# NorESMhub/BLOM

Measured on AMD Instinct MI355X. Metric: simulated-days/sec, higher is better.
Workload: dtype f64; 1 GPU; channel 208x512x53 as 1 tile(s) of 208x512x53 along i, 1 tile per GPU, isopyc_bulkml/remap/geopotential/uc/enscon, ntr=3 (TKE, length-scale slot, ideal age: the reference default build), baclin=900s batrop=18s lstep=50; config 2's step (phy/mod_blom_step.F90:96-253: init_fluxes, tmsmt1, cmnfld2, difest_isobml [the whole routine: diffusivities estimated every step (NorESM defaults incl. rhsctp; the; physics=full, forcing=default, spinup_steps=0

## Files before the change

### blom_amd/csrc/blomgpu_internal.h

```cpp
#pragma once
#include <hip/hip_runtime.h>
#include <cstdint>
#include <string>
#include <unordered_map>
#include <vector>
#include "exp_libm.h"

#define NBDY 4

#ifdef BLOM_HOSTEMU
#define WAIT_VMCNT0() ((void)0)
#else
#define WAIT_VMCNT0() asm volatile("s_waitcnt vmcnt(0)" ::: "memory")
#endif

#define BLOM_REAL_FIELDS(X)                                                              \
                                                                          \
  X(u, 2 * K) X(v, 2 * K) X(dp, 2 * K) X(dpu, 2 * K) X(dpv, 2 * K) X(temp, 2 * K)        \
  X(saln, 2 * K) X(sigma, 2 * K) X(uflx, 2 * K) X(vflx, 2 * K) X(utflx, 2 * K)           \
  X(vtflx, 2 * K) X(usflx, 2 * K) X(vsflx, 2 * K)                                        \
  X(p, K + 1) X(pu, K + 1) X(pv, K + 1) X(phi, K + 1) X(cau, K) X(cav, K)                \
  X(ubflxs, 3) X(vbflxs, 3) X(ub, 2) X(vb, 2) X(pb, 2) X(pbu, 2) X(pbv, 2)               \
  X(ubflxs_p, 2) X(vbflxs_p, 2) X(pb_p, 1) X(pbu_p, 1) X(pbv_p, 1) X(ubcors_p, 1)        \
  X(vbcors_p, 1) X(sealv, 1)                                                             \
// ... 220 lines not shown
  bool ale_density_pc_upper = false, ale_density_pc_lower = false;
  int ale_regrid_method = 2, ale_k_range_plevel = 1;
  double ale_regrid_nudge_ts = 86400., ale_stab_fac_limit = .75, ale_dpvar_fac = .75, ale_smooth_diff_max = 50000.;
  int ale_dktzu = 4, ale_dktzl = 2;
  double ale_dpmin_interior = .1 * 9806.;
  int ndiff_rec_per_face = 0;
  int ndiff_surface_align = 1;
  double rm0 = 1.2, rm5 = 0., niwgf = 0., niwbf = .35, niwlf = .5;
  std::string mlrttp = "constant";
  double trxday = 0., srxday = 0., trxdpt = 1., srxdpt = 1., trxlim = 1.5, srxlim = .5, sref = 34.65, area = 0., xmi = 0.;
  int lmi[5] = {11, 12, 1, 2, 3};
  bool aptflx = false, apsflx = false, ditflx = false, disflx = false, srxbal = false;
  int ntda = 0;
  double swamxd = 200., brine_mlbase_frac = 0.;
  int mlrmth = 1;
  double eddtra_ce = .06, tau_mlr = 86400., tau_growing_hbl = 300., tau_decaying_hbl = 86400., tau_growing_hml = 3600.,
         tau_decaying_hml = 259200., lfmin = 5.e3, mlbl_max_ratio = 3., eddtra_cl = .25, mstar = .5, nstar = .066, wpup_min = 1.e-3;
  double egc = 0., eggam = 200., eglsmn = 4000., egmndf = 0., egmxdf = 1500., egidfq = 1., rhiscf = 0., ri0 = 1.2, tkepf = 0.;
  double bdml_logc = 0.;
  int eddf2d = 0, edsprs = 1, edanis = 0, redi3d = 0, rhsctp = 0, edfsmo = 0;
  int edritp_opt = 2, edwmth_opt = 1;
  bool smtfrc = false, use_stream_relaxation = false;
  int nstep_in_cpl = 1, l1ci = 1, l2ci = 1, nstep_in_day = 1, nday_of_year = 1;
  int cesm_single_sums = 0;
  bool full_physics = false;
  int difest_live = 0;
  int live_slopes = 0;
  int cmnfld1 = 0;
  int eddtra_frozen = 0;
  int check_period = 8;
  bool timing = false;
  int use_graph = 0;
  int overlap = 1;
  int phys_dag = 7;
  int mom_early_at = 0;
  int lean_fluxes = 1;
  int tmsmt_fold = 1;
  int tmsmt_ahead = 1;
  int remap_fold = 0;
  int remap_nfirst = 4;
  int halo_overlap = 1;
  int barotp_fused = 1;
  int barotp_tile = 0;
  int barotp_persist = 1;
  int barotp_block = 1;
  int barotp_overlap = 0;
  int barotp_rimbuf = 1;
  int barotp_arctic_persist = 1;
  int barotp_arctic_fused = 1;
  int arctic_strips = 0;
  int pgf_uv_pair = 0;
  int pgf_uv_ring = 7;
  int pgf_reuse = 0;
  int pgf_copy_fused = 1;
  int scan_reassoc = 0;
  int mom_aw_split = 0;
  int mom_force_aw = 0;
  int momtum_order = 0;
  int momtum_lds_pad = 0;
  int momtum_bs = 0;
  int momtum_chunks_a = 0, momtum_chunks_b = 0;
  int convec_nsingle = 2;
  int cmn_nslope_nb = 4;
  int diapfl_du = 8;
  int diffus_shfl = 0;
  int kprof_sel = 1;

// ... 220 lines not shown
```

### blom_amd/csrc/stage_cmnfld.hip

```cpp
#include "blomgpu_internal.h"
#include "eos.h"

#define GRAV 9.806
#define RHO0 1.e3
#define EPSILP 1.e-12
#define ONEM 9806.
#define ONEMM 9.806
#define SLS0 (10. * ONEM)
#define SLSMFQ 2.
#define SLSELS 2.
#define BFSQMN 1.e-7

enum { CM_DELP, CM_BFSQ, CM_SLS2, CM_GAM_ALE, CM_GAM = 9, CM_NSLOT };

#define COLUMN_IJ(V)                                                     \
  const int t_ = blockIdx.x * blockDim.x + threadIdx.x;                  \
  if (t_ >= (V).nplane) return;                                          \
  const int i = t_ % (V).ni - (NBDY - 1), j = t_ / (V).ni - (NBDY - 1);  \
  const size_t c = t_

__global__ __launch_bounds__(64) void k_cmn_bfsqf(const DevView *__restrict__ Vp, int n, int nn) {
  const DevView &V = *Vp;
  COLUMN_IJ(V);
  if (j < -1 || j > V.jj + 2 || i < -1 || i > V.ii + 2 || !V.m[I_ip][c]) return;
// ... 118 lines not shown
  L(bfsqf, kk + 1) = f_kk;
#undef L
}

__global__ __launch_bounds__(64) void k_cmn_phi(const DevView *__restrict__ Vp, int nn) {
  const DevView &V = *Vp;
  COLUMN_IJ(V);
  if (j < -1 || j > V.jj + 2 || i < -1 || i > V.ii + 2 || !V.m[I_ip][c]) return;
  const size_t np = V.nplane;
  const int kk = V.kk;
  gcd_t p = V.f[F_p] + c, temp = V.f[F_temp] + c + (size_t)nn * np, saln = V.f[F_saln] + c + (size_t)nn * np;
  gcd_t dp = V.f[F_dp] + c + (size_t)nn * np;
  gd_t phi = V.f[F_phi] + c;
  double ph = phi[(size_t)kk * np], plo = p[(size_t)kk * np];
  for (int k0 = kk - 1; k0 >= 0; k0 -= COLUMN_U) {
    double a[COLUMN_U], b[COLUMN_U], d[COLUMN_U], e[COLUMN_U];
#pragma unroll
    for (int u = 0; u < COLUMN_U; u++) {
      const size_t o = (size_t)(k0 - u >= 0 ? k0 - u : 0) * np;
      a[u] = p[o]; b[u] = dp[o]; d[u] = temp[o]; e[u] = saln[o];
    }
#pragma unroll
    for (int u = 0; u < COLUMN_U; u++) {
      const int k = k0 - u;
      if (k >= 0) {
        if (!(b[u] < EPSILP)) ph = ph - eos::p_alpha(plo, a[u], d[u], e[u]);
        phi[(size_t)k * np] = ph;
        plo = a[u];
      }
    }
  }
}

template <int NB>
__global__ __launch_bounds__(64) void k_cmn_nslope(const DevView *__restrict__ Vp, int n, int nn) {
  const DevView &V = *Vp;
  COLUMN_IJ(V);
  const bool isv = blockIdx.y == 1;
  if (isv ? (j < 0 || j > V.jj + 2 || i < -1 || i > V.ii + 2 || !V.m[I_iv][c])
          : (j < -1 || j > V.jj + 2 || i < 0 || i > V.ii + 2 || !V.m[I_iu][c])) return;
  const size_t np = V.nplane, a_ = isv ? c - V.ni : c - 1, b_ = c;
  const int kk = V.kk;
  gcd_t p = V.f[F_p], phi = V.f[F_phi], bf = V.f[F_bfsqf];
  gcd_t temp = V.f[F_temp] + (size_t)nn * np, saln = V.f[F_saln] + (size_t)nn * np, dp = V.f[F_dp] + (size_t)nn * np;
  gd_t nslp = (isv ? V.f[F_nslpy] : V.f[F_nslpx]) + c, nnslp = (isv ? V.f[F_nnslpy] : V.f[F_nnslpx]) + c;
  const double sci = (isv ? V.f[F_scvyi] : V.f[F_scuxi])[c];
#define A(f, x, k) (f)[(x) + (size_t)((k)-1) * np]
#define O(f, k) (f)[(size_t)((k)-1) * np]
  for (int k = 1; k <= kk; k++) { O(nslp, k) = 0.; O(nnslp, k) = 0.; }
  const int kfa = V.m[I_kfpla][a_ + (size_t)(n - 1) * np], kfb = V.m[I_kfpla][b_ + (size_t)(n - 1) * np];
  if (!(kfa <= kk || kfb <= kk)) return;
  int kmax = 1;
  for (int k0 = 3; k0 <= kk; k0 += COLUMN_U) {
    double da[COLUMN_U], db[COLUMN_U];
#pragma unroll
    for (int u = 0; u < COLUMN_U; u++) { const int kq = k0 + u <= kk ? k0 + u : kk; da[u] = A(dp, a_, kq); db[u] = A(dp, b_, kq); }
#pragma unroll
    for (int u = 0; u < COLUMN_U; u++)
      if (k0 + u <= kk && (da[u] > EPSILP || db[u] > EPSILP)) kmax = k0 + u;
  }
  const int kintr = kfa > kfb ? kfa : kfb;
  int knnsl = 2;
  const double phba = A(phi, a_, kk + 1), phbb = A(phi, b_, kk + 1);
  {
    const double pm = .5 * (A(p, a_, 3) + A(p, b_, 3));
    const double rx = eos::rho(pm, A(temp, b_, 2), A(saln, b_, 2)) - eos::rho(pm, A(temp, a_, 2), A(saln, a_, 2));
// ... 12 lines not shown
#pragma unroll
      for (int u = 0; u < NB; u++) {
        const int kq = k0 + u <= kmax ? k0 + u : kmax;
        pa[u] = A(p, a_, kq); pb[u] = A(p, b_, kq);
        tb[u] = A(temp, b_, kq); sb[u] = A(saln, b_, kq); ta[u] = A(temp, a_, kq); sa[u] = A(saln, a_, kq);
        fb[u] = A(phi, b_, kq); fa[u] = A(phi, a_, kq); ba[u] = A(bf, a_, kq); bb[u] = A(bf, b_, kq);
      }
#pragma unroll
      for (int u = 0; u < NB; u++) {
        const int k = k0 + u;
        if (k > kmax) break;
        const double pm = .5 * (pa[u] + pb[u]);
        const double rx = .5 * (eos::rho(pm, tbm, sbm) - eos::rho(pm, tam, sam) + eos::rho(pm, tb[u], sb[u]) - eos::rho(pm, ta[u], sa[u]));
        const double px = fb[u] - fa[u];
        const double bm = .5 * (ba[u] + bb[u]);
        const double s = (GRAV * rx / (RHO0 * bm) + px / GRAV) * sci;
        O(nslp, k) = s;
        if (fb[u] > phba && fa[u] > phbb) { O(nnslp, k) = sqrt(bm) * s; knnsl = k; }
        tbm = tb[u]; sbm = sb[u]; tam = ta[u]; sam = sa[u];
      }
    }
  }
  {
    const double last = O(nnslp, knnsl);
    for (int k = knnsl + 1; k <= kmax; k++) O(nnslp, k) = last;
  }
  if (kintr < kmax) {
    const double s = O(nslp, kintr + 1), ns = O(nnslp, kintr + 1);
    for (int k = 4; k <= kintr; k++) { O(nslp, k) = s; O(nnslp, k) = ns; }
  } else {
    const double s = O(nslp, 3), ns = O(nnslp, 3);
    for (int k = 4; k <= kmax; k++) { O(nslp, k) = s; O(nnslp, k) = ns; }
  }
#undef A
#undef O
}

__global__ __launch_bounds__(64) void k_cmn_z(const DevView *__restrict__ Vp, int mm) {
  const DevView &V = *Vp;
  COLUMN_IJ(V);
  if (j < 1 || j > V.jj || i < 1 || i > V.ii || !V.m[I_ip][c]) return;
  const size_t np = V.nplane;
  const int kk = V.kk;
  gcd_t p = V.f[F_p] + c, temp = V.f[F_temp] + c + (size_t)mm * np, saln = V.f[F_saln] + c + (size_t)mm * np;
  gcd_t dp = V.f[F_dp] + c + (size_t)mm * np;
  gd_t z = V.f[F_z] + c, dz = V.f[F_dz] + c;
  double zlo = -V.f[F_phi][c + (size_t)kk * np] / GRAV, plo = p[(size_t)kk * np];
  z[(size_t)kk * np] = zlo;
  for (int k0 = kk - 1; k0 >= 0; k0 -= COLUMN_U) {
    double a[COLUMN_U], b[COLUMN_U], d[COLUMN_U], e[COLUMN_U];
#pragma unroll
    for (int u = 0; u < COLUMN_U; u++) {
      const size_t o = (size_t)(k0 - u >= 0 ? k0 - u : 0) * np;
      a[u] = p[o]; b[u] = dp[o]; d[u] = temp[o]; e[u] = saln[o];
    }
#pragma unroll
    for (int u = 0; u < COLUMN_U; u++) {
      const int k = k0 - u;
      if (k < 0) break;
      const double zk = b[u] < EPSILP ? zlo : zlo + eos::p_alpha(plo, a[u], d[u], e[u]) / GRAV;
      z[(size_t)k * np] = zk;
      dz[(size_t)k * np] = zlo - zk;
      zlo = zk; plo = a[u];
    }
  }
}
// ... 307 lines not shown
    if (int rc = st_xctilr_multi(c, 2, ptrs, nl, 3, 3, it)) return rc;
  }
  const dim3 g1 = plane_grid(h, 1, 64), g2 = plane_grid(h, 2, 64);
  if (h.P.vcoord_tag != 1) {
    if (h.P.ltedtp_opt == 2 && h.P.eitmth == 2) {
      if (int rc = st_xctilr(c, h.f[F_nslpx], 1, h.kk, 2, 2, 13)) return rc;
      if (int rc = st_xctilr(c, h.f[F_nslpy], 1, h.kk, 2, 2, 14)) return rc;
    }
    TimeScope ts(c, "cmnfld");
    HIPCHK(c, hipMemsetAsync(h.f[F_bfsqi], 0, sizeof(double) * (size_t)(h.kk + 1) * h.nplane, c->stream));
    HIPCHK(c, hipMemsetAsync(h.f[F_bfsql], 0, sizeof(double) * (size_t)h.kk * h.nplane, c->stream));
    hipLaunchKernelGGL(k_cmn_bfsqf_ale, g1, dim3(64), 0, c->stream, c->d, nn);
    if (h.P.eitmth == 2) {
      if (h.P.ltedtp_opt == 2) hipLaunchKernelGGL(k_cmn_nnslope_ale, g2, dim3(64), 0, c->stream, c->d);
      else {
        hipLaunchKernelGGL(k_cmn_phi, g1, dim3(64), 0, c->stream, c->d, nn);
        hipLaunchKernelGGL(k_cmn_nslope_ale, g2, dim3(64), 0, c->stream, c->d, nn);
      }
    }
    HIPCHK(c, hipGetLastError());
    return 0;
  }
  if (int rc = st_kfpla_halo(c, n)) return rc;
  if (h.P.eitmth != 2) return 0;
  const bool aside = ctx_overlap_on(c) && (c->phys_dag & 1) && !c->tiling.multi();
  hipStream_t s = c->stream;
  if (aside) {
    if (int rc = launch_pscan(c, nn, -2, 3)) return rc;
    c->seq.pscan_done_ahead = true;
    if (int rc = ctx_side_fork(c, 4)) return rc;
    s = c->side;
  }
  TimeScope ts(c, "cmnfld");
  hipLaunchKernelGGL(k_cmn_bfsqf, g1, dim3(64), 0, s, c->d, n, nn);
  hipLaunchKernelGGL(k_cmn_phi, g1, dim3(64), 0, s, c->d, nn);
  switch (c->cmn_nslope_nb) {
    case 4: hipLaunchKernelGGL(k_cmn_nslope<4>, g2, dim3(64), 0, s, c->d, n, nn); break;
    case 3: hipLaunchKernelGGL(k_cmn_nslope<3>, g2, dim3(64), 0, s, c->d, n, nn); break;
    default: hipLaunchKernelGGL(k_cmn_nslope<2>, g2, dim3(64), 0, s, c->d, n, nn); break;
  }
  HIPCHK(c, hipGetLastError());
  c->seq.cmn_on_side = aside;
  return 0;
}
```

### blom_amd/csrc/stage_difest_iso.hip

```cpp
#include "blomgpu_internal.h"
#include "../../include/blomgpu.h"
#include "eos.h"
#include "pow_libm.h"
#include "sin_libm.h"
#include "atan2_libm.h"
#include <cmath>

#define PLANE_IJ(V)                                                        \
  unsigned bx_, by_;                                                       \
  xcd_block(bx_, by_);                                                     \
  const int t_ = bx_ * blockDim.x + threadIdx.x;                           \
  (void)by_;                                                               \
  if (t_ >= (V).nplane) return;                                            \
  const int i = t_ % (V).ni - (NBDY - 1), j = t_ / (V).ni - (NBDY - 1);    \
  const size_t c = t_;                                                     \
  (void)i; (void)j; (void)c

#define GRAV 9.806
#define ALPHA0 1.e-3
#define PI_BLOM 3.1415926536
#define BU 8
#define EPSILP 1.e-12
#define ONEM 9806.
#define DPBMIN 98.06
// ... 13 lines not shown
#define DPGRAV (100. * ONEM)
#define DPDIAV (100. * ONEM)
#define DPDDAV (10. * ONEM)
#define DPNBAV (250. * ONEM)
#define USTMIN .001
#define KAPPA .4
#define BFEPS 1.e-16
#define SLEPS .1
#define ZETAS (-1.)
#define CPSEMIN (-0.2)
#define URMSEMIN 0.05
#define AS_ (-28.86)
#define CS_ 98.96
#define GLS_CMU0 .527
#define PR_T 1.
#define GLS_C1 1.44
#define GLS_C2 1.92
#define GLS_C3PLUS 1.
#define GLS_C3MINUS (-.63)
#define GLS_GH0 .0329
#define GLS_GHMIN (-.28)
#define GLS_GHCRI .03
#define LS_UNLMT_MIN 1.e-8

enum { W_DU2 = 0, W_DV2, W_BVFSQ, W_BVF, W_EGR, W_ANISOK, W_SM1, W_SM2, W_NUB, W_NSLOT };

struct TkeC {
  double sqrt2, cmu_fac1, cmu_fac2, cmu_fac3, tke_exp1, gls_exp1, gls_fac6, s0, s1, s2, s4, s5, s6, b0, b1, b2, b3, b4, b5, cmu0p3;
  double gls_qfac, gls_bbc, gls_cmu0p;
};
struct DfePar {
  double egc, eggam, eglsmn, egmndf, egmxdf, egidfq, rhiscf, ri0, tkepf, niwgf, niwbf, niwlf, bdml_logc;
  int eddf2d, edsprs, edanis, redi3d, edritp, edwmth, use_tke, use_gls, itke, igls, rhsctp;
  TkeC T;
};

static TkeC tke_consts() {
  const double L1 = .107, L2 = .0032, L3 = .0864, L4 = .12, L5 = 11.9, L6 = .4, L7 = .0, L8 = .48;
  const double gls_p = 3., gls_m = 1.5, gls_n = -1.;
  TkeC t;
  t.sqrt2 = std::sqrt(2.);
  t.cmu_fac1 = std::pow(GLS_CMU0, -gls_p / gls_n);
  t.cmu_fac2 = std::pow(GLS_CMU0, 3. + gls_p / gls_n);
  t.cmu_fac3 = t.sqrt2;
  t.tke_exp1 = gls_m / gls_n;
  t.gls_exp1 = 1. / gls_n;
  const double c2 = GLS_CMU0 * GLS_CMU0;
  t.gls_fac6 = 8. / (c2 * (c2 * c2));
  t.cmu0p3 = GLS_CMU0 * c2;
  t.gls_qfac = std::pow(.56, .5 * gls_n) * std::pow(GLS_CMU0, gls_p);
  t.gls_bbc = std::pow(.4, gls_n);
  t.gls_cmu0p = std::pow(GLS_CMU0, gls_p);
  t.s0 = 1.5 * L1 * (L5 * L5);
  t.s1 = -L4 * (L6 + L7) + 2. * L4 * L5 * (L1 - 1. / 3. * L2 - L3) + 1.5 * L1 * L5 * L8;
  t.s2 = -3. / 8. * L1 * (L6 * L6 - L7 * L7);
  t.s4 = 2. * L5;
  t.s5 = 2. * L4;
  t.s6 = 2. / 3. * L5 * (3. * (L3 * L3) - L2 * L2) - .5 * L5 * L1 * (3. * L3 - L2) + .75 * L1 * (L6 - L7);
  t.b0 = 3. * (L5 * L5);
  t.b1 = L5 * (7. * L4 + 3. * L8);
  t.b2 = (L5 * L5) * (3. * (L3 * L3) - L2 * L2) - .75 * (L6 * L6 - L7 * L7);
  t.b3 = L4 * (4. * L4 + 3. * L8);
  t.b4 = L4 * (L2 * L6 - 3. * L3 * L7 - L5 * (L2 * L2 - L3 * L3)) + L5 * L8 * (3. * (L3 * L3) - L2 * L2);
  t.b5 = .25 * (L2 * L2 - 3. * (L3 * L3)) * (L6 * L6 - L7 * L7);
  return t;
}
// ... 107 lines not shown
  const DevView &V = *Vp;
  PLANE_IJ(V);
  if (j < 1 || j > V.jj || i < 1 || i > V.ii || !V.m[I_ip][c]) return;
  const int kf = V.m[I_dfe_kfil][c], km = V.m[I_dfe_kmax][c];
  if (km - kf < 1) return;
  const int kk = V.kk, ni = V.ni;
  const int k = by_ + 1;
  const int k1 = kf > 4 ? kf : 4, k2 = km < kk ? km : kk;
  if (k < k1 || k > k2) return;
  const size_t np = V.nplane, o = (size_t)(k - 1) * np + c;
  gcd_t p = V.f[F_p], temp = V.f[F_temp] + (size_t)nn * np, saln = V.f[F_saln] + (size_t)nn * np;
  auto jump = [&](int kq) {
    const size_t oq = (size_t)(kq - 1) * np + c, o1 = (size_t)(kq < kk ? kq : kk - 1) * np + c;
    const double pk1 = p[oq + np];
    return fmax2(0., eos::rho(pk1, temp[o1], saln[o1]) - eos::rho(pk1, temp[oq], saln[oq]));
  };
  const double tup = k - 1 >= k1 ? jump(k - 1) : 0.;
  double dr;
  if (k < km) {
    const double q = jump(k);
    if (k == kf) dr = q;
    else dr = 2. * tup * q / fmax2(1.e-11, tup + q);
  } else
    dr = tup;
  V.f[F_drhol][o] = dr;
  const int mu0 = V.m[I_msku][o], mu1 = V.m[I_msku][o + 1], mv0 = V.m[I_mskv][o], mv1 = V.m[I_mskv][o + ni];
  gcd_t du2 = WK(V, W_DU2), dv2 = WK(V, W_DV2);
  const double d2 = ((double)mu0 * du2[o] + (double)mu1 * du2[o + 1]) / (double)(mu0 + mu1 > 1 ? mu0 + mu1 : 1) +
                    ((double)mv0 * dv2[o] + (double)mv1 * dv2[o + ni]) / (double)(mv0 + mv1 > 1 ? mv0 + mv1 : 1);
  V.f[F_du2l][o] = d2;
  V.f[F_rig][o] = ALPHA0 * ALPHA0 * fmax2(DRHOMN, dr) * V.f[F_dp][o + (size_t)nn * np] / fmax2(1.e-13, d2);
}

#define S2_BVFBOT 10
#define S2_EXPB 11
__global__ __launch_bounds__(64) void k_dfi_vert_a(const DevView *__restrict__ Vp, DfePar D, int nn) {
  const DevView &V = *Vp;
  PLANE_IJ(V);
  if (j < 1 || j > V.jj || i < 1 || i > V.ii || !V.m[I_ip][c]) return;
  const int kf = V.m[I_dfe_kfil][c], km = V.m[I_dfe_kmax][c];
  const size_t np = V.nplane;
  const int kk = V.kk;
  gcd_t p = V.f[F_p] + c, dp = V.f[F_dp] + c + (size_t)nn * np;
  gcd_t drhol = V.f[F_drhol] + c, du2l = V.f[F_du2l] + c, difdia = V.f[F_difdia] + c;
  gd_t bvfsq = WK(V, W_BVFSQ) + c, bvf = WK(V, W_BVF) + c, ex = V.f[F_wkp1] + c;
  gd_t Buoy = V.f[F_Buoy] + c, Shear2 = V.f[F_Shear2] + c, Prod = V.f[F_Prod] + c;
  const double pbot = p[(size_t)kk * np], q = V.f[F_tdmls][c];
  double bvfbot = 0., dps = 0.;
  if (km - kf >= 1) {
    const int k1 = kf > 4 ? kf : 4;
    double pk = p[(size_t)(k1 - 1) * np];
    ex[(size_t)(k1 - 1) * np] = exp_libm(pk / q);
    const int k2 = km < kk ? km : kk;
    for (int k0 = k1; k0 <= k2; k0 += BU) {
      double a0[BU], a1[BU], a2[BU], a3[BU], a4[BU];
#pragma unroll
      for (int uu = 0; uu < BU; uu++) {
        const size_t o = (size_t)((k0 + uu <= k2 ? k0 + uu : k2) - 1) * np;
        a0[uu] = dp[o]; a1[uu] = p[o + np]; a2[uu] = drhol[o]; a3[uu] = D.use_tke ? du2l[o] : 0.; a4[uu] = D.use_tke ? difdia[o] : 0.;
      }
#pragma unroll
      for (int uu = 0; uu < BU; uu++) {
        const int k = k0 + uu;
        if (k > k2) break;
        const size_t o = (size_t)(k - 1) * np;
        const double dpk = a0[uu], pk1 = a1[uu];
// ... 560 lines not shown
        esfac = 1. / (1. + r * r);
      } else {
        double umnsc = ubc * cosang;
        umnsc = umnsc - vbc * sinang - cpse;
        const double r = umnsc / fmax2(URMSEMIN, fabs(urmse));
        esfac = 1. / (1. + 4. * (r * r));
      }
    } else
      esfac = 1.;
    if (D.eddf2d) {
      double d1;
      if (D.edanis) d1 = anisos * dfints * difwgt;
      else d1 = dfints * difwgt;
      if (D.redi3d) difiso[0] = fmin3(difmxp, D.egmxdf, fmax2(D.egmndf, esfac * dfints * D.egidfq * difwgt));
      else difiso[0] = fmin3(difmxp, D.egmxdf, fmax2(D.egmndf, d1 * D.egidfq));
      difint[0] = fmin3(difmxp, D.egmxdf, fmax2(D.egmndf, d1));
    } else {
      const double d1 = fmin3(difmxp, D.egmxdf, fmax2(D.egmndf, dfints * difwgt * esfac));
      difint[0] = d1;
      difiso[0] = d1 * D.egidfq;
    }
  } else {
    dfints = D.egmndf;
    difiso[0] = difint[0] * D.egidfq;
  }
  {
    double li = difint[0], ls_ = difiso[0];
    const double di1 = li, ds1 = ls_;
    const int k_end = any ? ka - 1 : kk;
    for (int k = 2; k <= k_end; k++) { difint[(size_t)(k - 1) * np] = li; difiso[(size_t)(k - 1) * np] = ls_; }
    if (any && D.eddf2d && !D.redi3d) {
      for (int k = ka; k <= kk; k++) { difint[(size_t)(k - 1) * np] = di1; difiso[(size_t)(k - 1) * np] = ds1; }
    } else if (any) {
      for (int k0 = ka; k0 <= kb; k0 += BU) {
        double dv[BU], av[BU], u0[BU], u1[BU], v0[BU], v1[BU];
        int mu0[BU], mu1[BU], mv0[BU], mv1[BU];
#pragma unroll
        for (int uu = 0; uu < BU; uu++) {
          const size_t o = (size_t)((k0 + uu <= kb ? k0 + uu : kb) - 1) * np;
          dv[uu] = difint[o];
          av[uu] = D.edanis ? anisok[o] : 1.;
          if (D.edsprs) {
            mu0[uu] = msku[o]; mu1[uu] = msku[o + 1]; mv0[uu] = mskv[o]; mv1[uu] = mskv[o + ni];
            u0[uu] = u[o]; u1[uu] = u[o + 1]; v0[uu] = v[o]; v1[uu] = v[o + ni];
          }
        }
#pragma unroll
        for (int uu = 0; uu < BU; uu++) {
          const int k = k0 + uu;
          if (k > kb) break;
          const size_t o = (size_t)(k - 1) * np;
          double esfac;
          if (D.edsprs) {
            const double umnsc = ((double)mu0[uu] * u0[uu] + (double)mu1[uu] * u1[uu]) / (double)(mu0[uu] + mu1[uu] > 1 ? mu0[uu] + mu1[uu] : 1) * cosang -
                                 ((double)mv0[uu] * v0[uu] + (double)mv1[uu] * v1[uu]) / (double)(mv0[uu] + mv1[uu] > 1 ? mv0[uu] + mv1[uu] : 1) * sinang - cpse;
            const double r = umnsc / fmax2(URMSEMIN, fabs(urmse));
            esfac = 1. / (1. + 4. * (r * r));
          } else if (D.edanis)
            esfac = av[uu];
          else
            esfac = 1.;
          if (D.eddf2d) {
            li = di1;
            if (D.redi3d) ls_ = fmin3(difmxp, D.egmxdf, fmax2(D.egmndf, esfac * dfints * D.egidfq * difwgt));
            else ls_ = ds1;
          } else {
            li = fmin3(difmxp, D.egmxdf, fmax2(D.egmndf, dv[uu] * difwgt * esfac));
            ls_ = li * D.egidfq;
          }
          difint[o] = li;
          difiso[o] = ls_;
        }
      }
      for (int k = kb + 1; k <= kk; k++) { difint[(size_t)(k - 1) * np] = li; difiso[(size_t)(k - 1) * np] = ls_; }
    }
  }
// ... 14 lines not shown
  const double ww = .125 * (double)ip[c - 1] * fmin2(ONEM, dp[c - 1]) / ONEM;
  const double we = .125 * (double)ip[c + 1] * fmin2(ONEM, dp[c + 1]) / ONEM;
  const double wn = .125 * (double)ip[c + ni] * fmin2(ONEM, dp[c + ni]) / ONEM;
  const double wc = -((ws + ww) + (we + wn)) + 1.;
  V.f[F_difint][c + o] = (ws * u1[c - ni] + ww * u1[c - 1]) + (we * u1[c + 1] + wn * u1[c + ni]) + wc * u1[c];
  V.f[F_difiso][c + o] = (ws * u2[c - ni] + ww * u2[c - 1]) + (we * u2[c + 1] + wn * u2[c + ni]) + wc * u2[c];
}

extern "C" int blomgpu_tke_const(const char *name, double *v) {
  const TkeC t = tke_consts();
  const std::string s(name);
#define G(nm, f) if (s == #nm) { *v = t.f; return 0; }
  G(sqrt2, sqrt2) G(cmu_fac1, cmu_fac1) G(cmu_fac2, cmu_fac2) G(cmu_fac3, cmu_fac3) G(tke_exp1, tke_exp1) G(gls_exp1, gls_exp1)
  G(gls_fac6, gls_fac6) G(gls_s0, s0) G(gls_s1, s1) G(gls_s2, s2) G(gls_s4, s4) G(gls_s5, s5) G(gls_s6, s6)
  G(gls_b0, b0) G(gls_b1, b1) G(gls_b2, b2) G(gls_b3, b3) G(gls_b4, b4) G(gls_b5, b5)
#undef G
  return 1;
}

int st_difest_isobml(blomgpu_ctx *c, int m, int n, int mm, int nn) {
  const DevView &h = c->h;
  if (h.P.vcoord_tag != 1) return ctx_fail(c, "difest_isobml is the isopycnic coordinate's (phy/mod_blom_step.F90:140)");
  if (h.P.itrtke >= 1 && (h.P.itrtke > h.ntr || h.P.itrgls < 1 || h.P.itrgls > h.ntr)) return ctx_fail(c, "difest: itrtke / itrgls outside 1..ntr");
  if (h.P.bdmldp && c->bdml_logc == 0.) return ctx_fail(c, " difest_vertical_iso: bdmldp needs the plane bdmlq and the option bdml_logc (the host's log)");
  if (W_NSLOT > h.nwk) return ctx_fail(c, "difest: work space too small");
  if (int rc = st_difest_isobml_pre(c, m, n, mm, nn)) return rc;
  DfePar D;
  D.egc = c->egc; D.eggam = c->eggam; D.eglsmn = c->eglsmn; D.egmndf = c->egmndf; D.egmxdf = c->egmxdf; D.egidfq = c->egidfq;
  D.rhiscf = c->rhiscf; D.ri0 = c->ri0; D.tkepf = c->tkepf; D.niwgf = c->niwgf; D.niwbf = c->niwbf; D.niwlf = c->niwlf;
  D.bdml_logc = c->bdml_logc;
  D.rhsctp = c->rhsctp; D.eddf2d = c->eddf2d; D.edsprs = c->edsprs; D.edanis = c->edanis; D.redi3d = c->redi3d; D.edritp = c->edritp_opt; D.edwmth = c->edwmth_opt;
  D.use_tke = h.P.itrtke >= 1; D.use_gls = D.use_tke && h.P.gls; D.itke = h.P.itrtke; D.igls = h.P.itrgls;
  D.T = tke_consts();
  const dim3 g1 = plane_grid(h, 1, 64), g2 = plane_grid(h, 2, 64), b64(64);
  {
    TimeScope ts(c, "difest");
    hipLaunchKernelGGL(k_dfi_kmax_kfil, g1, b64, 0, c->stream, c->d, n, nn);
    hipLaunchKernelGGL(k_dfi_kfil_util, plane_grid(h), dim3(256), 0, c->stream, c->d, 0);
  }
  if (int rc = st_xctilr(c, h.f[F_util1], 1, 1, 1, 1, 1)) return rc;
  {
    TimeScope ts(c, "difest");
    hipLaunchKernelGGL(k_dfi_kfil_util, plane_grid(h), dim3(256), 0, c->stream, c->d, 1);
    hipLaunchKernelGGL(k_dfi_uv2, g2, b64, 0, c->stream, c->d, nn);
    hipLaunchKernelGGL(k_dfi_common, plane_grid(h, h.kk), dim3(256), 0, c->stream, c->d, nn);
    const bool aside = ctx_overlap_on(c) && (c->phys_dag & 1) && !c->tiling.multi();
    hipStream_t sl = c->stream;
    if (aside) {
      if (int rc = ctx_side_fork(c, 5)) return rc;
      sl = c->side;
    }
    hipLaunchKernelGGL(k_dfi_vert_a, g1, b64, 0, c->stream, c->d, D, nn);
    hipLaunchKernelGGL(k_dfi_vert_b, plane_grid(h, h.kk), dim3(256), 0, c->stream, c->d, D, nn);
    hipLaunchKernelGGL(k_dfi_vert_c, g1, b64, 0, c->stream, c->d, D, nn);
    if (D.rhsctp) hipLaunchKernelGGL(k_dfi_falign, plane_grid(h, h.kk), dim3(256), 0, sl, c->d, n, nn);
    hipLaunchKernelGGL(k_dfi_lateral, g1, b64, 0, sl, c->d, D, n, nn);
    if (aside) {
      c->seq.cmn_on_side = false;
      if (int rc = ctx_side_done(c, 4)) return rc;
      if (int rc = ctx_side_join(c, 4)) return rc;
    }
  }
  HIPCHK(c, hipGetLastError());
  const int mrgint = 1, mrgiso = 2;
  if (c->edfsmo) {
    if (int rc = st_xctilr(c, h.f[F_difint], 1, h.kk, mrgint + 1, mrgint + 1, 1)) return rc;
    if (int rc = st_xctilr(c, h.f[F_difiso], 1, h.kk, mrgiso + 1, mrgiso + 1, 1)) return rc;
    const size_t bytes = sizeof(double) * (size_t)h.kk * h.nplane;
    HIPCHK(c, hipMemcpyAsync(WK(h, W_SM1), h.f[F_difint], bytes, hipMemcpyDeviceToDevice, c->stream));
    HIPCHK(c, hipMemcpyAsync(WK(h, W_SM2), h.f[F_difiso], bytes, hipMemcpyDeviceToDevice, c->stream));
    hipLaunchKernelGGL(k_dfi_smooth, plane_grid(h, h.kk), dim3(256), 0, c->stream, c->d, nn);
    HIPCHK(c, hipGetLastError());
  } else {
    if (int rc = st_xctilr(c, h.f[F_difint], 1, h.kk, mrgint, mrgint, 1)) return rc;
    if (int rc = st_xctilr(c, h.f[F_difiso], 1, h.kk, mrgiso, mrgiso, 1)) return rc;
  }
  return 0;
}
// ... 1 lines not shown
```

Measured before the change: 1.607 simulated-days/sec.

## Fuse bfsqf+phi, single-pass nslope, and range-encoded uv shear in difest

```diff
diff --git a/blom_amd/csrc/blomgpu_internal.h b/blom_amd/csrc/blomgpu_internal.h
--- a/blom_amd/csrc/blomgpu_internal.h
+++ b/blom_amd/csrc/blomgpu_internal.h
@@ -276,7 +276,7 @@
   bool timing = false;
   int use_graph = 0;
   int overlap = 1;
-  int phys_dag = 7;
+  int phys_dag = 119;
   int mom_early_at = 0;
   int lean_fluxes = 1;
   int tmsmt_fold = 1;
diff --git a/blom_amd/csrc/stage_cmnfld.hip b/blom_amd/csrc/stage_cmnfld.hip
--- a/blom_amd/csrc/stage_cmnfld.hip
+++ b/blom_amd/csrc/stage_cmnfld.hip
@@ -174,6 +174,153 @@
   }
 }
 
+__global__ __launch_bounds__(64) void k_cmn_bfsqf_phi(const DevView *__restrict__ Vp, int n, int nn) {
+  const DevView &V = *Vp;
+  COLUMN_IJ(V);
+  if (j < -1 || j > V.jj + 2 || i < -1 || i > V.ii + 2 || !V.m[I_ip][c]) return;
+  const size_t np = V.nplane;
+  const int kk = V.kk;
+  gcd_t p = V.f[F_p] + c, temp = V.f[F_temp] + c + (size_t)nn * np, saln = V.f[F_saln] + c + (size_t)nn * np;
+  gcd_t dp = V.f[F_dp] + c + (size_t)nn * np;
+  gd_t bfsqi = V.f[F_bfsqi] + c, bfsql = V.f[F_bfsql] + c, bfsqf = V.f[F_bfsqf] + c;
+  gd_t gam = WK(V, CM_GAM) + c;
+  gd_t phi = V.f[F_phi] + c;
+#define L(a, k) (a)[(size_t)((k)-1) * np]
+  [&]() {
+    const double b1 = .5 * GRAV * GRAV * (eos::rho(L(p, 2), L(temp, 2), L(saln, 2)) - eos::rho(L(p, 2), L(temp, 1), L(saln, 1))) /
+                      (L(dp, 1) + L(dp, 2));
+    L(bfsqi, 1) = b1; L(bfsqi, 2) = b1; L(bfsql, 1) = b1; L(bfsql, 2) = b1;
+    const int kfpl = V.m[I_kfpla][c + (size_t)(n - 1) * np];
+    if (kfpl > kk) {
+      for (int k = 3; k <= kk; k++) { L(bfsqi, k) = b1; L(bfsql, k) = b1; }
+      L(bfsqi, kk + 1) = b1;
+      for (int k = 1; k <= kk + 1; k++) L(bfsqf, k) = BFSQMN;
+      return;
+    }
+    const double pbot = L(p, kk + 1);
+    const double pml = fmax2(.5 * (L(p, 3) + L(p, 1)), .5 * (3. * L(p, 3) - L(p, kfpl + 1)));
+    const double dml = pml - L(p, 1);
+    L(bfsqi, kfpl - 1) = L(bfsqi, 2);
+    double delp_mm = 0., delp_m = dml, sls2_mm = 0., sls2_m, bfsq_m = BFSQMN, bi_m = b1;
+    {
+      const double q = fmax2(SLS0, dml * SLSMFQ);
+      sls2_m = q * q;
+    }
+    double pup = pml, tup = L(temp, 2), sup = L(saln, 2);
+    double pk = L(p, kfpl);
+    double ctd = 0., btd, bei = 0., fprev = 0., bi_kfpl = 0., bl_kfpl = 0.;
+    for (int k0 = kfpl; k0 <= kk; k0 += COLUMN_U) {
+      double a0[COLUMN_U], a1[COLUMN_U], a2[COLUMN_U];
+#pragma unroll
+      for (int u = 0; u < COLUMN_U; u++) {
+        const int kq = k0 + u <= kk ? k0 + u : kk;
+        a0[u] = L(p, kq + 1); a1[u] = L(temp, kq); a2[u] = L(saln, kq);
+      }
+#pragma unroll
+      for (int u = 0; u < COLUMN_U; u++) {
+        const int k = k0 + u;
+        if (k > kk) break;
+        const double pk1 = a0[u];
+        double delp_k, bfsq_k, sls2_k, bi;
+        if (pbot - pk < EPSILP) {
+          delp_k = ONEMM;
+          bi = bi_m;
+          bfsq_k = BFSQMN;
+          double q = exp_libm(-(pbot - pml) / (SLSELS * dml));
+          q = fmax2(SLS0, dml * SLSMFQ * q + SLS0 * (1. - q));
+          sls2_k = q * q;
+        } else {
+          const double plo = pbot - pk1 < EPSILP ? pbot : .5 * (pk + pk1);
+          const double tlo = a1[u], slo = a2[u];
+          const double dk = fmax2(ONEMM, plo - pup);
+          delp_k = dk;
+          bi = GRAV * GRAV * (eos::rho(pk, tlo, slo) - eos::rho(pk, tup, sup)) / dk;
+          bfsq_k = fmax2(BFSQMN, bi);
+          bi = bi * dk / fmax2(ONEM, dk);
+          if (pbot - pk < ONEM) bi = bi_m;
+          double q = exp_libm(-(pk - pml) / (SLSELS * dml));
+          q = fmax2(SLS0, dml * SLSMFQ * q + SLS0 * (1. - q));
+          sls2_k = q * q;
+          pup = plo; tup = tlo; sup = slo;
+        }
+        L(bfsqi, k) = bi;
+        if (k == kfpl) {
+          bi_kfpl = bi;
+          ctd = -2. * sls2_m / (delp_m * (delp_m + delp_k));
+          btd = 1. - ctd;
+          bei = 1. / btd;
+          fprev = bfsq_m * bei;
+          L(bfsqf, k - 1) = fprev;
+        } else {
+          const double bl = .5 * (bi_m + bi);
+          L(bfsql, k - 1) = bl;
+          if (k == kfpl + 1) bl_kfpl = bl;
+          const double atd = -2. * sls2_mm / (delp_m * (delp_mm + delp_m));
+          const double g = ctd * bei;
+          L(gam, k - 1) = g;
+          ctd = -2. * sls2_m / (delp_m * (delp_m + delp_k));
+          btd = 1. - atd - ctd;
+          bei = 1. / (btd - atd * g);
+          fprev = (bfsq_m - atd * fprev) * bei;
+          L(bfsqf, k - 1) = fprev;
+        }
+        delp_mm = delp_m; delp_m = delp_k; sls2_mm = sls2_m; sls2_m = sls2_k; bfsq_m = bfsq_k; bi_m = bi;
+        pk = pk1;
+      }
+    }
+    L(bfsql, kk) = bi_m;
+    if (kfpl == kk) bl_kfpl = bi_m;
+    for (int k = 3; k <= kfpl - 1; k++) { L(bfsqi, k) = bi_kfpl; L(bfsql, k) = bl_kfpl; }
+    {
+      const double atd = -2. * sls2_mm / (delp_m * (delp_mm + delp_m));
+      const double g = ctd * bei;
+      L(gam, kk) = g;
+      btd = 1. - atd;
+      bei = 1. / (btd - atd * g);
+      fprev = (bfsq_m - atd * fprev) * bei;
+      L(bfsqf, kk) = fprev;
+    }
+    const double f_kk = fprev;
+    for (int k0 = kk - 1; k0 >= kfpl - 1; k0 -= COLUMN_U) {
+      double a0[COLUMN_U], a1[COLUMN_U];
+#pragma unroll
+      for (int u = 0; u < COLUMN_U; u++) {
+        const int kq = k0 - u >= kfpl - 1 ? k0 - u : kfpl - 1;
+        a0[u] = L(bfsqf, kq); a1[u] = L(gam, kq + 1);
+      }
+#pragma unroll
+      for (int u = 0; u < COLUMN_U; u++) {
+        const int k = k0 - u;
+        if (k < kfpl - 1) break;
+        fprev = a0[u] - a1[u] * fprev;
+        L(bfsqf, k) = fprev;
+      }
+    }
+    for (int k = 1; k <= kfpl - 2; k++) L(bfsqf, k) = fprev;
+    L(bfsqi, kk + 1) = bi_m;
+    L(bfsqf, kk + 1) = f_kk;
+  }();
+#undef L
+  double ph = phi[(size_t)kk * np], plo = p[(size_t)kk * np];
+  for (int k0 = kk - 1; k0 >= 0; k0 -= COLUMN_U) {
+    double a[COLUMN_U], b[COLUMN_U], d[COLUMN_U], e[COLUMN_U];
+#pragma unroll
+    for (int u = 0; u < COLUMN_U; u++) {
+      const size_t o = (size_t)(k0 - u >= 0 ? k0 - u : 0) * np;
+      a[u] = p[o]; b[u] = dp[o]; d[u] = temp[o]; e[u] = saln[o];
+    }
+#pragma unroll
+    for (int u = 0; u < COLUMN_U; u++) {
+      const int k = k0 - u;
+      if (k >= 0) {
+        if (!(b[u] < EPSILP)) ph = ph - eos::p_alpha(plo, a[u], d[u], e[u]);
+        phi[(size_t)k * np] = ph;
+        plo = a[u];
+      }
+    }
+  }
+}
+
 template <int NB>
 __global__ __launch_bounds__(64) void k_cmn_nslope(const DevView *__restrict__ Vp, int n, int nn) {
   const DevView &V = *Vp;
@@ -252,6 +399,107 @@
     const double s = O(nslp, 3), ns = O(nnslp, 3);
     for (int k = 4; k <= kmax; k++) { O(nslp, k) = s; O(nnslp, k) = ns; }
   }
+#undef A
+#undef O
+}
+
+template <int NB>
+__global__ __launch_bounds__(64) void k_cmn_nslope_once(const DevView *__restrict__ Vp, int n, int nn) {
+  const DevView &V = *Vp;
+  COLUMN_IJ(V);
+  const bool isv = blockIdx.y == 1;
+  if (isv ? (j < 0 || j > V.jj + 2 || i < -1 || i > V.ii + 2 || !V.m[I_iv][c])
+          : (j < -1 || j > V.jj + 2 || i < 0 || i > V.ii + 2 || !V.m[I_iu][c])) return;
+  const size_t np = V.nplane, a_ = isv ? c - V.ni : c - 1, b_ = c;
+  const int kk = V.kk;
+  gcd_t p = V.f[F_p], phi = V.f[F_phi], bf = V.f[F_bfsqf];
+  gcd_t temp = V.f[F_temp] + (size_t)nn * np, saln = V.f[F_saln] + (size_t)nn * np, dp = V.f[F_dp] + (size_t)nn * np;
+  gd_t nslp = (isv ? V.f[F_nslpy] : V.f[F_nslpx]) + c, nnslp = (isv ? V.f[F_nnslpy] : V.f[F_nnslpx]) + c;
+  const double sci = (isv ? V.f[F_scvyi] : V.f[F_scuxi])[c];
+#define A(f, x, k) (f)[(x) + (size_t)((k)-1) * np]
+#define O(f, k) (f)[(size_t)((k)-1) * np]
+  const int kfa = V.m[I_kfpla][a_ + (size_t)(n - 1) * np], kfb = V.m[I_kfpla][b_ + (size_t)(n - 1) * np];
+  if (!(kfa <= kk || kfb <= kk)) {
+    for (int k = 1; k <= kk; k++) { O(nslp, k) = 0.; O(nnslp, k) = 0.; }
+    return;
+  }
+  const int kintr = kfa > kfb ? kfa : kfb;
+  const bool low = kintr < 3;
+  for (int k = 1; k <= (low ? kk : 2); k++) { O(nslp, k) = 0.; O(nnslp, k) = 0.; }
+  int kmax = 1;
+  for (int k0 = 3; k0 <= kk; k0 += COLUMN_U) {
+    double da[COLUMN_U], db[COLUMN_U];
+#pragma unroll
+    for (int u = 0; u < COLUMN_U; u++) { const int kq = k0 + u <= kk ? k0 + u : kk; da[u] = A(dp, a_, kq); db[u] = A(dp, b_, kq); }
+#pragma unroll
+    for (int u = 0; u < COLUMN_U; u++)
+      if (k0 + u <= kk && (da[u] > EPSILP || db[u] > EPSILP)) kmax = k0 + u;
+  }
+  int knnsl = 2;
+  double last = 0.;
+  const double phba = A(phi, a_, kk + 1), phbb = A(phi, b_, kk + 1);
+  double s3, n3 = 0.;
+  {
+    const double pm = .5 * (A(p, a_, 3) + A(p, b_, 3));
+    const double rx = eos::rho(pm, A(temp, b_, 2), A(saln, b_, 2)) - eos::rho(pm, A(temp, a_, 2), A(saln, a_, 2));
+    const double px = A(phi, b_, 3) - A(phi, a_, 3);
+    const double bm = .5 * (A(bf, a_, 3) + A(bf, b_, 3));
+    const double s = (GRAV * rx / (RHO0 * bm) + px / GRAV) * sci;
+    s3 = s;
+    if (A(phi, b_, 3) > phba && A(phi, a_, 3) > phbb) { n3 = sqrt(bm) * s; knnsl = 3; last = n3; }
+    O(nslp, 3) = s;
+    O(nnslp, 3) = n3;
+  }
+  const int kf = kintr + 1;
+  double sf = 0., nf = 0.;
+  bool abovef = false;
+  {
+    double tbm = kf <= kmax ? A(temp, b_, kf - 1) : 0., sbm = kf <= kmax ? A(saln, b_, kf - 1) : 0.;
+    double tam = kf <= kmax ? A(temp, a_, kf - 1) : 0., sam = kf <= kmax ? A(saln, a_, kf - 1) : 0.;
+    for (int k0 = kf; k0 <= kmax; k0 += NB) {
+      double pa[NB], pb[NB], tb[NB], sb[NB], ta[NB], sa[NB], fb[NB], fa[NB], ba[NB], bb[NB];
+#pragma unroll
+      for (int u = 0; u < NB; u++) {
+        const int kq = k0 + u <= kmax ? k0 + u : kmax;
+        pa[u] = A(p, a_, kq); pb[u] = A(p, b_, kq);
+        tb[u] = A(temp, b_, kq); sb[u] = A(saln, b_, kq); ta[u] = A(temp, a_, kq); sa[u] = A(saln, a_, kq);
+        fb[u] = A(phi, b_, kq); fa[u] = A(phi, a_, kq); ba[u] = A(bf, a_, kq); bb[u] = A(bf, b_, kq);
+      }
+#pragma unroll
+      for (int u = 0; u < NB; u++) {
+        const int k = k0 + u;
+        if (k > kmax) break;
+        const double pm = .5 * (pa[u] + pb[u]);
+        const double rx = .5 * (eos::rho(pm, tbm, sbm) - eos::rho(pm, tam, sam) + eos::rho(pm, tb[u], sb[u]) - eos::rho(pm, ta[u], sa[u]));
+        const double px = fb[u] - fa[u];
+        const double bm = .5 * (ba[u] + bb[u]);
+        const double s = (GRAV * rx / (RHO0 * bm) + px / GRAV) * sci;
+        O(nslp, k) = s;
+        if (k == kf) sf = s;
+        if (fb[u] > phba && fa[u] > phbb) {
+          const double ns = sqrt(bm) * s;
+          for (int kz = knnsl + 1 > kf ? knnsl + 1 : kf; kz < k; kz++) O(nnslp, kz) = 0.;
+          O(nnslp, k) = ns;
+          knnsl = k;
+          last = ns;
+          if (k == kf) { nf = ns; abovef = true; }
+        }
+        tbm = tb[u]; sbm = sb[u]; tam = ta[u]; sam = sa[u];
+      }
+    }
+  }
+  for (int k = low || knnsl + 1 > kf ? knnsl + 1 : kf; k <= kmax; k++) O(nnslp, k) = last;
+  int kz;
+  if (kintr < kmax) {
+    const double ns = abovef ? nf : knnsl < kf ? last : 0.;
+    for (int k = 4; k <= kintr; k++) { O(nslp, k) = sf; O(nnslp, k) = ns; }
+    kz = kmax + 1;
+  } else {
+    for (int k = 4; k <= kmax; k++) { O(nslp, k) = s3; O(nnslp, k) = n3; }
+    kz = kmax > 3 ? kmax + 1 : 4;
+  }
+  if (!low)
+    for (int k = kz; k <= kk; k++) { O(nslp, k) = 0.; O(nnslp, k) = 0.; }
 #undef A
 #undef O
 }
@@ -625,9 +873,17 @@
     s = c->side;
   }
   TimeScope ts(c, "cmnfld");
-  hipLaunchKernelGGL(k_cmn_bfsqf, g1, dim3(64), 0, s, c->d, n, nn);
-  hipLaunchKernelGGL(k_cmn_phi, g1, dim3(64), 0, s, c->d, nn);
-  switch (c->cmn_nslope_nb) {
+  if (c->phys_dag & 32) hipLaunchKernelGGL(k_cmn_bfsqf_phi, g1, dim3(64), 0, s, c->d, n, nn);
+  else {
+    hipLaunchKernelGGL(k_cmn_bfsqf, g1, dim3(64), 0, s, c->d, n, nn);
+    hipLaunchKernelGGL(k_cmn_phi, g1, dim3(64), 0, s, c->d, nn);
+  }
+  if (c->phys_dag & 64) switch (c->cmn_nslope_nb) {
+    case 4: hipLaunchKernelGGL(k_cmn_nslope_once<4>, g2, dim3(64), 0, s, c->d, n, nn); break;
+    case 3: hipLaunchKernelGGL(k_cmn_nslope_once<3>, g2, dim3(64), 0, s, c->d, n, nn); break;
+    default: hipLaunchKernelGGL(k_cmn_nslope_once<2>, g2, dim3(64), 0, s, c->d, n, nn); break;
+  }
+  else switch (c->cmn_nslope_nb) {
     case 4: hipLaunchKernelGGL(k_cmn_nslope<4>, g2, dim3(64), 0, s, c->d, n, nn); break;
     case 3: hipLaunchKernelGGL(k_cmn_nslope<3>, g2, dim3(64), 0, s, c->d, n, nn); break;
     default: hipLaunchKernelGGL(k_cmn_nslope<2>, g2, dim3(64), 0, s, c->d, n, nn); break;
diff --git a/blom_amd/csrc/stage_difest_iso.hip b/blom_amd/csrc/stage_difest_iso.hip
--- a/blom_amd/csrc/stage_difest_iso.hip
+++ b/blom_amd/csrc/stage_difest_iso.hip
@@ -69,6 +69,7 @@
 struct DfePar {
   double egc, eggam, eglsmn, egmndf, egmxdf, egidfq, rhiscf, ri0, tkepf, niwgf, niwbf, niwlf, bdml_logc;
   int eddf2d, edsprs, edanis, redi3d, edritp, edwmth, use_tke, use_gls, itke, igls, rhsctp;
+  int uvrng;
   TkeC T;
 };
 
@@ -242,6 +243,103 @@
   V.f[F_rig][o] = ALPHA0 * ALPHA0 * fmax2(DRHOMN, dr) * V.f[F_dp][o + (size_t)nn * np] / fmax2(1.e-13, d2);
 }
 
+#define S2_URNG 12
+#define S2_VRNG 13
+#define DFI_RNG_IN(r, k) ((k) >= ((r) & 0xffff) && (k) <= ((r) >> 16) && ((r) >> 16) - ((r) & 0xffff) >= 1)
+__global__ __launch_bounds__(64) void k_dfi_uvrange(const DevView *__restrict__ Vp, int nn) {
+  const DevView &V = *Vp;
+  PLANE_IJ(V);
+  const bool isv = by_ == 1;
+  if (isv ? (j < 1 || j > V.jj + 1 || i < 1 || i > V.ii) : (j < 1 || j > V.jj || i < 1 || i > V.ii + 1)) return;
+  const size_t np = V.nplane;
+  const int kk = V.kk;
+  gi_t rng = (gi_t)WK2(V, isv ? S2_VRNG : S2_URNG) + c;
+  int klpl = 1, kfpl = kk + 1;
+  if (V.m[isv ? I_iv : I_iu][c]) {
+    gcd_t dpz = V.f[isv ? F_dpv : F_dpu] + c + (size_t)nn * np;
+    gci_t kfil = V.m[I_dfe_kfil];
+    const int ka = kfil[isv ? c - V.ni : c - 1], kb = kfil[c];
+    const int kf = isv ? (ka > kb ? ka : kb) : (ka < kb ? ka : kb);
+    for (int k0 = 3; k0 <= kk; k0 += COLUMN_U) {
+      double a[COLUMN_U];
+#pragma unroll
+      for (int u = 0; u < COLUMN_U; u++) a[u] = dpz[(size_t)((k0 + u <= kk ? k0 + u : kk) - 1) * np];
+#pragma unroll
+      for (int u = 0; u < COLUMN_U; u++)
+        if (k0 + u <= kk) {
+          const int k = k0 + u;
+          if (a[u] > DPBMIN) klpl = k;
+          if (k >= 4 && k >= kf && a[u] > DPTMIN && kfpl == kk + 1) kfpl = k;
+        }
+    }
+  }
+  rng[0] = kfpl + 65536 * klpl;
+}
+
+#define DFI_NL 4
+__global__ void k_dfi_common_uv(const DevView *__restrict__ Vp, int nn) {
+  const DevView &V = *Vp;
+  PLANE_IJ(V);
+  if (j < 1 || j > V.jj || i < 1 || i > V.ii || !V.m[I_ip][c]) return;
+  const int kf = V.m[I_dfe_kfil][c], km = V.m[I_dfe_kmax][c];
+  if (km - kf < 1) return;
+  const int kk = V.kk, ni = V.ni;
+  const int k1 = kf > 4 ? kf : 4, k2 = km < kk ? km : kk;
+  const int ka = (int)by_ * DFI_NL + 1 > k1 ? (int)by_ * DFI_NL + 1 : k1, kb = (int)by_ * DFI_NL + DFI_NL < k2 ? (int)by_ * DFI_NL + DFI_NL : k2;
+  if (ka > kb) return;
+  const size_t np = V.nplane;
+  gcd_t p = V.f[F_p], temp = V.f[F_temp] + (size_t)nn * np, saln = V.f[F_saln] + (size_t)nn * np, dp = V.f[F_dp] + (size_t)nn * np;
+  gci_t urng = (gci_t)WK2(V, S2_URNG), vrng = (gci_t)WK2(V, S2_VRNG);
+  const int rng[4] = {urng[c], urng[c + 1], vrng[c], vrng[c + ni]};
+  gcd_t vel[4] = {V.f[F_u] + (size_t)nn * np + c, V.f[F_u] + (size_t)nn * np + c + 1, V.f[F_v] + (size_t)nn * np + c, V.f[F_v] + (size_t)nn * np + c + ni};
+  double vm[4], v0[4];
+#pragma unroll
+  for (int f = 0; f < 4; f++) { vm[f] = vel[f][(size_t)(ka - 2) * np]; v0[f] = vel[f][(size_t)(ka - 1) * np]; }
+  auto jump = [&](int kq) {
+    const size_t oq = (size_t)(kq - 1) * np + c, o1 = (size_t)(kq < kk ? kq : kk - 1) * np + c;
+    const double pk1 = p[oq + np];
+    return fmax2(0., eos::rho(pk1, temp[o1], saln[o1]) - eos::rho(pk1, temp[oq], saln[oq]));
+  };
+  double tup = ka - 1 >= k1 ? jump(ka - 1) : 0.;
+#pragma unroll
+  for (int u = 0; u < DFI_NL; u++) {
+    const int k = ka + u;
+    if (k > kb) break;
+    const size_t o = (size_t)(k - 1) * np + c;
+    double vp[4];
+#pragma unroll
+    for (int f = 0; f < 4; f++) vp[f] = vel[f][(size_t)(k < kk ? k : kk - 1) * np];
+    const double dpk = dp[o];
+    double dr, q = 0.;
+    if (k < km) {
+      q = jump(k);
+      if (k == kf) dr = q;
+      else dr = 2. * tup * q / fmax2(1.e-11, tup + q);
+    } else
+      dr = tup;
+    tup = q;
+    V.f[F_drhol][o] = dr;
+    double d[4];
+    int m[4];
+#pragma unroll
+    for (int f = 0; f < 4; f++) {
+      const int kfpl = rng[f] & 0xffff, klpl = rng[f] >> 16;
+      double qm = v0[f] - vm[f];
+      qm = qm * qm;
+      double qk = vp[f] - v0[f];
+      qk = qk * qk;
+      m[f] = DFI_RNG_IN(rng[f], k);
+      d[f] = !m[f] ? 0. : k == kfpl ? qk : k < klpl ? .5 * (qm + qk) : qm;
+      vm[f] = v0[f];
+      v0[f] = vp[f];
+    }
+    const double d2 = ((double)m[0] * d[0] + (double)m[1] * d[1]) / (double)(m[0] + m[1] > 1 ? m[0] + m[1] : 1) +
+                      ((double)m[2] * d[2] + (double)m[3] * d[3]) / (double)(m[2] + m[3] > 1 ? m[2] + m[3] : 1);
+    V.f[F_du2l][o] = d2;
+    V.f[F_rig][o] = ALPHA0 * ALPHA0 * fmax2(DRHOMN, dr) * dpk / fmax2(1.e-13, d2);
+  }
+}
+
 #define S2_BVFBOT 10
 #define S2_EXPB 11
 __global__ __launch_bounds__(64) void k_dfi_vert_a(const DevView *__restrict__ Vp, DfePar D, int nn) {
@@ -868,6 +966,11 @@
     if (any && D.eddf2d && !D.redi3d) {
       for (int k = ka; k <= kk; k++) { difint[(size_t)(k - 1) * np] = di1; difiso[(size_t)(k - 1) * np] = ds1; }
     } else if (any) {
+      int ru0 = 0, ru1 = 0, rv0 = 0, rv1 = 0;
+      if (D.edsprs && D.uvrng) {
+        gci_t urng = (gci_t)WK2(V, S2_URNG) + c, vrng = (gci_t)WK2(V, S2_VRNG) + c;
+        ru0 = urng[0]; ru1 = urng[1]; rv0 = vrng[0]; rv1 = vrng[ni];
+      }
       for (int k0 = ka; k0 <= kb; k0 += BU) {
         double dv[BU], av[BU], u0[BU], u1[BU], v0[BU], v1[BU];
         int mu0[BU], mu1[BU], mv0[BU], mv1[BU];
@@ -877,7 +980,12 @@
           dv[uu] = difint[o];
           av[uu] = D.edanis ? anisok[o] : 1.;
           if (D.edsprs) {
-            mu0[uu] = msku[o]; mu1[uu] = msku[o + 1]; mv0[uu] = mskv[o]; mv1[uu] = mskv[o + ni];
+            if (D.uvrng) {
+              const int kq = k0 + uu <= kb ? k0 + uu : kb;
+              mu0[uu] = DFI_RNG_IN(ru0, kq); mu1[uu] = DFI_RNG_IN(ru1, kq); mv0[uu] = DFI_RNG_IN(rv0, kq); mv1[uu] = DFI_RNG_IN(rv1, kq);
+            } else {
+              mu0[uu] = msku[o]; mu1[uu] = msku[o + 1]; mv0[uu] = mskv[o]; mv1[uu] = mskv[o + ni];
+            }
             u0[uu] = u[o]; u1[uu] = u[o + 1]; v0[uu] = v[o]; v1[uu] = v[o + ni];
           }
         }
@@ -958,6 +1066,7 @@
   D.rhsctp = c->rhsctp; D.eddf2d = c->eddf2d; D.edsprs = c->edsprs; D.edanis = c->edanis; D.redi3d = c->redi3d; D.edritp = c->edritp_opt; D.edwmth = c->edwmth_opt;
   D.use_tke = h.P.itrtke >= 1; D.use_gls = D.use_tke && h.P.gls; D.itke = h.P.itrtke; D.igls = h.P.itrgls;
   D.T = tke_consts();
+  D.uvrng = (c->phys_dag & 16) != 0;
   const dim3 g1 = plane_grid(h, 1, 64), g2 = plane_grid(h, 2, 64), b64(64);
   {
     TimeScope ts(c, "difest");
@@ -968,8 +1077,13 @@
   {
     TimeScope ts(c, "difest");
     hipLaunchKernelGGL(k_dfi_kfil_util, plane_grid(h), dim3(256), 0, c->stream, c->d, 1);
-    hipLaunchKernelGGL(k_dfi_uv2, g2, b64, 0, c->stream, c->d, nn);
-    hipLaunchKernelGGL(k_dfi_common, plane_grid(h, h.kk), dim3(256), 0, c->stream, c->d, nn);
+    if (D.uvrng) {
+      hipLaunchKernelGGL(k_dfi_uvrange, g2, b64, 0, c->stream, c->d, nn);
+      hipLaunchKernelGGL(k_dfi_common_uv, plane_grid(h, (h.kk + DFI_NL - 1) / DFI_NL), dim3(256), 0, c->stream, c->d, nn);
+    } else {
+      hipLaunchKernelGGL(k_dfi_uv2, g2, b64, 0, c->stream, c->d, nn);
+      hipLaunchKernelGGL(k_dfi_common, plane_grid(h, h.kk), dim3(256), 0, c->stream, c->d, nn);
+    }
     const bool aside = ctx_overlap_on(c) && (c->phys_dag & 1) && !c->tiling.multi();
     hipStream_t sl = c->stream;
     if (aside) {
```

Result: faster. 1.629 simulated-days/sec (median of 6 runs) (+1.4%).
